# narayanan2004/GraphMat

Measured on AMD Instinct MI355X. Metric: GTEPS (edges/s) per iter + achieved HBM GB/s, PageRank RMAT-26, higher is better.
Workload: dtype f32

## Files before the change

graphmat_amd/csrc/gm_graph.hip:

```cpp
#include <string.h>
#include <cstring>

#include <hip/hip_runtime.h>
#include <rocprim/rocprim.hpp>

#include <algorithm>
#include <cmath>
#include <vector>

#include "gm_internal.hpp"

namespace gm {

int g_short_row = GM_SHORT_ROW;
int g_giant_row = 0;
int g_rank_cap = 0;
int g_rank_by = 0;
int g_tile_min_row = GM_TILE_MIN_ROW;
int g_tile_balance = 1;
int g_long_mid = 0;
int g_sweep_slices = 1;
int g_sort_tile_lists = 1;
int g_sweep_border_factor = 4;
int g_sweep_stream_weight = 300;
int g_sweep_stream = 1;
int g_sweep_waves = 16;
int g_sweep_fold_share = 50;
int g_sweep_long_row = 0;
int g_sweep_acc_limit = GM_SWEEP_ACC_ROWS, g_sweep_long_limit = GM_SWEEP_LONG_SLOTS;
int g_own_wave_row = 4096;
int g_col_tiles = 0;

constexpr int kT = 256;
inline int grid_for(int64_t n) { return (int)((n + kT - 1) / kT); }

__global__ void __launch_bounds__(kT)
k_validate_ids(const int32_t* __restrict__ src, const int32_t* __restrict__ dst, int64_t nnz, int lo, int hi,
               unsigned long long* __restrict__ bad ) {
  const int64_t e = (int64_t)blockIdx.x * kT + threadIdx.x;
  bool b = false;
  if (e < nnz) {
    const int s = src[e], d = dst[e];
    b = s < lo || s > hi || d < lo || d > hi;
  }
  const unsigned long long m = __ballot(b);
  if (m && (threadIdx.x & 63) == __ffsll((long long)m) - 1) {
    atomicAdd(&bad[0], (unsigned long long)__popcll(m));
    atomicMin(&bad[1], (unsigned long long)e + 1ull);
  }
}
// ... 1073 lines not shown
  const int W = nwaves;
  const int FW = fold_waves;
  const uint32_t g0 = grp_first[b], g1 = grp_first[b + 1] - ((skip_groups != nullptr && b < nskip_blk) ? skip_groups[b] : 0u);
  auto cost = [&](uint32_t g_) -> unsigned long long {
    const unsigned long long rows = (gbase[g_ + 1] - gbase[g_]) / 64u + 1u;
    return (gblk != nullptr && (gblk[g_] & 0x80000000u)) ? (rows * (unsigned)stream_weight + 99ull) / 100ull : rows;
  };
  unsigned long long total = 0;
  for (uint32_t g = g0; g < g1; g++) total += cost(g);
  const unsigned long long units = (unsigned long long)(W - FW) * 100ull + (unsigned long long)FW * (unsigned)fold_share;
  uint32_t g = g0;
  unsigned long long acc = 0, share = 0;
  for (int w = 0; w < W; w++) {
    wfirst[(size_t)b * (WS + 1) + w] = g;
    wrow[(size_t)b * (WS + 1) + w] = gbase[g] >> 6;
    share += w >= W - FW ? (unsigned)fold_share : 100u;
    const unsigned long long want = total * share / units;
    while (g < g1 && acc + (cost(g) + 1u) / 2u <= want) { acc += cost(g); g++; }
  }
  for (int w = W; w <= WS; w++) {
    wfirst[(size_t)b * (WS + 1) + w] = g1;
    wrow[(size_t)b * (WS + 1) + w] = gbase[g1] >> 6;
  }
}
__global__ void __launch_bounds__(kT)
k_sweep_long_starts(const unsigned long long* __restrict__ key, int64_t n, int nslices, size_t nent, uint32_t* __restrict__ lps) {
  const size_t e = (size_t)blockIdx.x * kT + threadIdx.x;
  if (e > nent) return;
  if (e == nent) { lps[e] = (uint32_t)n; return; }
  const size_t b = e / GM_SWEEP_LONG_SLOTS;
  const unsigned long long vw = b / (size_t)nslices, slice = b % (size_t)nslices, j = e % GM_SWEEP_LONG_SLOTS;
  const unsigned long long want = (vw << 23) | (slice << 16) | j;
  int64_t lo = 0, hi = n;
  while (lo < hi) { const int64_t mid = (lo + hi) >> 1; if (key[mid] >= want) hi = mid; else lo = mid + 1; }
  lps[e] = (uint32_t)lo;
}
__global__ void __launch_bounds__(kT)
k_sweep_long_fill(const unsigned long long* __restrict__ key_sorted, const uint32_t* __restrict__ pos_sorted, int64_t n, const int32_t* __restrict__ colidx,
                  const uint32_t* __restrict__ vals, SweepSlices sl, uint32_t* __restrict__ lcol, uint32_t* __restrict__ lval) {
  const int64_t i = (int64_t)blockIdx.x * kT + threadIdx.x;
  if (i >= n) return;
  const uint32_t p = pos_sorted[i];
  lcol[i] = sweep_entry_of(sl, (int)((key_sorted[i] >> 16) & 127ull), colidx[p]);
  if (lval) lval[i] = vals[p];
}
__global__ void __launch_bounds__(kT)
// ... 249 lines not shown
    GM_TRY_HIP(hipMemcpyAsync(pstart.as<uint32_t>() + npieces, &ne32, 4, hipMemcpyHostToDevice, s));
    {
      std::vector<int32_t> h(nblk + 1);
      GM_TRY_HIP(hipMemcpyAsync(h.data(), bfirst.p, (nblk + 1) * 4, hipMemcpyDeviceToHost, s));
      GM_TRY_HIP(hipStreamSynchronize(s));
      h[nblk] = (int32_t)npieces;
      for (int64_t b = (int64_t)nblk - 1; b >= 0; b--) if (h[b] < 0) h[b] = h[b + 1];
      GM_TRY_HIP(hipMemcpyAsync(bfirst.p, h.data(), (nblk + 1) * 4, hipMemcpyHostToDevice, s));
      GM_TRY_HIP(hipStreamSynchronize(s));
    }
    head.free(); pidx.free();
    DevBuf pk_in, pk_out, pid_in, sp;
    if ((rc = pk_in.alloc((size_t)npieces * 8)) || (rc = pk_out.alloc((size_t)npieces * 8)) || (rc = pid_in.alloc((size_t)npieces * 4)) || (rc = sp.alloc((size_t)npieces * 4))) return rc;
    hipLaunchKernelGGL(k_sweep_piece_keys, dim3(grid_for((int64_t)npieces)), dim3(kT), 0, s, (const uint32_t*)pstart.as<uint32_t>(), (const uint32_t*)pblk.as<uint32_t>(), npieces,
                       pk_in.as<unsigned long long>(), pid_in.as<uint32_t>());
    if ((rc = sweep_sort_pairs(pk_in.as<unsigned long long>(), pk_out.as<unsigned long long>(), pid_in.as<uint32_t>(), sp.as<uint32_t>(), (size_t)npieces,
                               16 + bits_for((uint32_t)nblk), s)))
      return rc;
    pk_in.free(); pk_out.free(); pid_in.free(); pblk.free();
    DevBuf ng, grp_first;
    if ((rc = ng.alloc((nblk + 1) * 4)) || (rc = grp_first.alloc((nblk + 1) * 4))) return rc;
    GM_TRY_HIP(hipMemsetAsync(ng.p, 0, (nblk + 1) * 4, s));
    hipLaunchKernelGGL(k_sweep_block_groups, dim3(grid_for((int64_t)nblk)), dim3(kT), 0, s, (const int32_t*)bfirst.as<int32_t>(), (int)nblk, ng.as<uint32_t>());
    if (g_sweep_stream != 0) {
      const int nsblk = 256 * TS;
      DevBuf sflag, siota, scnt, slen, kin, vin, srows_;
      DevBuf& sgroups = st_sgroups;
      if ((rc = sflag.alloc((size_t)nrows)) || (rc = siota.alloc((size_t)nrows * 4)) || (rc = st_srow.alloc((size_t)nrows * 4 + 4)) || (rc = scnt.alloc(16))) return rc;
      hipLaunchKernelGGL(k_stream_flag, dim3(grid_for(nrows)), dim3(kT), 0, s, rowptr, nrows, whole->view.short_row, sflag.as<unsigned char>());
      hipLaunchKernelGGL(k_sweep_iota, dim3(grid_for(nrows)), dim3(kT), 0, s, siota.as<int32_t>(), nrows);
      tb = 0;
      GM_TRY_HIP(rocprim::select(nullptr, tb, siota.as<int32_t>(), sflag.as<unsigned char>(), st_srow.as<int32_t>(), scnt.as<unsigned int>(), (size_t)nrows, s));
      if ((rc = tmp.alloc(tb + 256))) return rc;
      GM_TRY_HIP(rocprim::select(tmp.p, tb, siota.as<int32_t>(), sflag.as<unsigned char>(), st_srow.as<int32_t>(), scnt.as<unsigned int>(), (size_t)nrows, s));
      GM_TRY_HIP(hipMemcpyAsync(&st_nshort, scnt.p, 4, hipMemcpyDeviceToHost, s));
      GM_TRY_HIP(hipStreamSynchronize(s));
      sflag.free(); siota.free();
      if (st_nshort > 0) {
        if ((rc = slen.alloc(((size_t)st_nshort + 1) * 4)) || (rc = st_soff.alloc(((size_t)st_nshort + 1) * 4))) return rc;
        GM_TRY_HIP(hipMemsetAsync(slen.p, 0, ((size_t)st_nshort + 1) * 4, s));
        hipLaunchKernelGGL(k_sweep_lens, dim3(grid_for((int)st_nshort)), dim3(kT), 0, s, (const int32_t*)st_srow.as<int32_t>(), (int)st_nshort, rowptr, slen.as<uint32_t>());
        if ((rc = sweep_excl_scan(slen.as<uint32_t>(), st_soff.as<uint32_t>(), (size_t)st_nshort + 1, s))) return rc;
        GM_TRY_HIP(hipMemcpyAsync(&st_edges, st_soff.as<uint32_t>() + st_nshort, 4, hipMemcpyDeviceToHost, s));
        GM_TRY_HIP(hipStreamSynchronize(s));
        slen.free();
      }
      st_nbins = (int)(((unsigned long long)st_edges + GM_STREAM_BIN - 1) / GM_STREAM_BIN);
// ... 16 lines not shown
        GM_TRY_HIP(hipMemcpyAsync(&st_rows_total, st_rowbase.as<uint32_t>() + nsblk, 4, hipMemcpyDeviceToHost, s));
        hipLaunchKernelGGL(k_stream_add_groups, dim3(grid_for(nsblk)), dim3(kT), 0, s, (const uint32_t*)sgroups.as<uint32_t>(), nsblk, ng.as<uint32_t>());
        hipLaunchKernelGGL(k_stream_bin_rows, dim3(grid_for(st_nbins + 1)), dim3(kT), 0, s, (const uint32_t*)st_soff.as<uint32_t>(), (int)st_nshort, st_nbins, st_binrow.as<uint32_t>());
        hipLaunchKernelGGL(k_stream_chunks, dim3(grid_for((int64_t)st_nbins * TS)), dim3(kT), 0, s, (const unsigned long long*)st_keys.as<unsigned long long>(), st_edges, TS, st_nbins,
                           (const uint32_t*)st_first.as<uint32_t>(), (const uint32_t*)st_rowbase.as<uint32_t>(), st_chunk.as<uint32_t>());
        GM_TRY_HIP(hipGetLastError());
        GM_TRY_HIP(hipStreamSynchronize(s));
        if ((rc = st_inv.alloc((size_t)st_rows_total * 64 * 2 + 64))) return rc;
        GM_TRY_HIP(hipMemsetAsync(st_inv.p, 0xff, (size_t)st_rows_total * 64 * 2 + 64, s));
        st_built = true;
      }
    }
    if ((rc = sweep_excl_scan(ng.as<uint32_t>(), grp_first.as<uint32_t>(), nblk + 1, s))) return rc;
    GM_TRY_HIP(hipMemcpyAsync(&ngroups, grp_first.as<uint32_t>() + nblk, 4, hipMemcpyDeviceToHost, s));
    GM_TRY_HIP(hipStreamSynchronize(s));
    DevBuf gsize, gb64, gq0, gblk;
    if ((rc = gsize.alloc(((size_t)ngroups + 1) * 8)) || (rc = gb64.alloc(((size_t)ngroups + 1) * 8)) || (rc = gq0.alloc(((size_t)ngroups + 1) * 4)) ||
        (rc = gblk.alloc(((size_t)ngroups + 1) * 4)) || (rc = gbase.alloc(((size_t)ngroups + 1) * 4)))
      return rc;
    GM_TRY_HIP(hipMemsetAsync(gsize.p, 0, ((size_t)ngroups + 1) * 8, s));
    hipLaunchKernelGGL(k_sweep_group_sizes, dim3((unsigned)nblk), dim3(64), 0, s, (const int32_t*)bfirst.as<int32_t>(), (const uint32_t*)grp_first.as<uint32_t>(),
                       (const uint32_t*)sp.as<uint32_t>(), (const uint32_t*)pstart.as<uint32_t>(), gsize.as<unsigned long long>(), gq0.as<uint32_t>(), gblk.as<uint32_t>(),
                       st_built ? (const uint32_t*)st_first.as<uint32_t>() : (const uint32_t*)nullptr, 256 * TS);
    if ((rc = sweep_excl_scan(gsize.as<unsigned long long>(), gb64.as<unsigned long long>(), (size_t)ngroups + 1, s))) return rc;
    GM_TRY_HIP(hipMemcpyAsync(&nentries, gb64.as<unsigned long long>() + ngroups, 8, hipMemcpyDeviceToHost, s));
    GM_TRY_HIP(hipStreamSynchronize(s));
    if (nentries >= (1ull << 32)) return GM_OK;
    hipLaunchKernelGGL(k_sweep_narrow, dim3(grid_for((int64_t)ngroups + 1)), dim3(kT), 0, s, (const unsigned long long*)gb64.as<unsigned long long>(), (size_t)ngroups + 1,
                       gbase.as<uint32_t>());
    gsize.free(); gb64.free();
    if ((rc = scol.alloc(((size_t)nentries + 64 * 64) * 4)) || (rc = wrow.alloc(nblk * 17 * 4)) || (rc = wfirst.alloc(nblk * 17 * 4))) return rc;
    if (vals && ((rc = sval.alloc(((size_t)nentries + 64 * 64) * 4)) || (rc = spos.alloc(((size_t)nentries + 64) * 4)))) return rc;
    hipLaunchKernelGGL(k_sweep_fill, dim3(65536), dim3(kT), 0, s, ngroups, (const uint32_t*)gbase.as<uint32_t>(), (const uint32_t*)gq0.as<uint32_t>(),
                       (const uint32_t*)gblk.as<uint32_t>(), (const int32_t*)bfirst.as<int32_t>(), (const uint32_t*)sp.as<uint32_t>(), (const uint32_t*)pstart.as<uint32_t>(),
                       (const uint16_t*)pslot16.as<uint16_t>(), mpos, colidx, vals, sl, TS, (const int*)rowmin.as<int>(), scol.as<uint32_t>(),
                       vals ? sval.as<uint32_t>() : (uint32_t*)nullptr, vals ? spos.as<uint32_t>() : (uint32_t*)nullptr);
    if (st_built)
      hipLaunchKernelGGL(k_stream_fill, dim3(65536), dim3(kT), 0, s, ngroups, (const uint32_t*)gbase.as<uint32_t>(), (const uint32_t*)gq0.as<uint32_t>(),
                         (const uint32_t*)gblk.as<uint32_t>(), (const uint32_t*)st_first.as<uint32_t>(), (const uint32_t*)st_rowbase.as<uint32_t>(),
                         (const unsigned long long*)st_keys.as<unsigned long long>(), (const uint32_t*)st_idx.as<uint32_t>(), (const uint32_t*)st_spos.as<uint32_t>(), colidx, vals, sl, TS,
                         scol.as<uint32_t>(), vals ? sval.as<uint32_t>() : (uint32_t*)nullptr, vals ? spos.as<uint32_t>() : (uint32_t*)nullptr, st_inv.as<uint16_t>());
    hipLaunchKernelGGL(k_sweep_wave_ranges, dim3((unsigned)((nblk + 63) / 64)), dim3(64), 0, s, (const uint32_t*)grp_first.as<uint32_t>(), (int)nblk,
                       (const uint32_t*)gbase.as<uint32_t>(), wfirst.as<uint32_t>(), wrow.as<uint32_t>(), nlong > 0 ? g_sweep_fold_share : 100,
                       (int)std::min(8, (((per_wg_long + nsets - 1) / nsets) + 63) / 64), (g_sweep_waves == 12 || g_sweep_waves == 8) ? g_sweep_waves : 16,
                       st_built ? (const uint32_t*)st_sgroups.as<uint32_t>() : (const uint32_t*)nullptr, 256 * TS);
    if (st_built) {
      if ((rc = st_wrow.alloc(nblk * 17 * 4)) || (rc = st_wfirst.alloc(nblk * 17 * 4))) return rc;
      hipLaunchKernelGGL(k_sweep_wave_ranges, dim3((unsigned)((nblk + 63) / 64)), dim3(64), 0, s, (const uint32_t*)grp_first.as<uint32_t>(), (int)nblk,
                         (const uint32_t*)gbase.as<uint32_t>(), st_wfirst.as<uint32_t>(), st_wrow.as<uint32_t>(), nlong > 0 ? g_sweep_fold_share : 100,
                         (int)std::min(8, (((per_wg_long + nsets - 1) / nsets) + 63) / 64), 16, (const uint32_t*)nullptr, 0, (const uint32_t*)gblk.as<uint32_t>(), g_sweep_stream_weight);
    }
    GM_TRY_HIP(hipGetLastError());
    GM_TRY_HIP(hipStreamSynchronize(s));
  } else {
    if ((rc = gbase.alloc(64)) || (rc = wrow.alloc(nblk * 17 * 4)) || (rc = wfirst.alloc(nblk * 17 * 4)) || (rc = scol.alloc(64 * 64 * 4))) return rc;
    GM_TRY_HIP(hipMemsetAsync(scol.p, 0xff, 64 * 64 * 4, s));
    if (vals) {
      if ((rc = sval.alloc(64 * 64 * 4))) return rc;
      GM_TRY_HIP(hipMemsetAsync(sval.p, 0, 64 * 64 * 4, s));
    }
    GM_TRY_HIP(hipMemsetAsync(gbase.p, 0, 64, s));
    GM_TRY_HIP(hipMemsetAsync(wfirst.p, 0, nblk * 17 * 4, s));
    GM_TRY_HIP(hipMemsetAsync(wrow.p, 0, nblk * 17 * 4, s));
    GM_TRY_HIP(hipStreamSynchronize(s));
  }
  DevBuf gcol, gval, gdst, gslice, gpos;
  int64_t ngiant_edges = 0;
  if (whole->view.ngiant > 0 && whole->view.giant_edges > 0 && whole->view.giant_edges < ((int64_t)1 << 32)) {
    const int64_t ge = whole->view.giant_edges;
    DevBuf gk_in, gk_out, gp_in, gp_out, gd_in, gd_out;
    if ((rc = gk_in.alloc((size_t)ge)) || (rc = gk_out.alloc((size_t)ge)) || (rc = gp_in.alloc((size_t)ge * 4)) || (rc = gp_out.alloc((size_t)ge * 4)) ||
        (rc = gd_in.alloc((size_t)ge * 4)) || (rc = gd_out.alloc((size_t)ge * 4)) || (rc = gslice.alloc((GM_MAX_SLICES + 2) * 4)))
      return rc;
// ... 1042 lines not shown
```

graphmat_amd/csrc/gm_programs.hip:

```cpp
#include <limits.h>
#include <math.h>

#include <string>

#include "GraphMatRuntime.h"
#include "gm_internal.hpp"

#define HD __host__ __device__

namespace gm {

extern int g_short_row, g_giant_row, g_rank_by, g_rank_cap, g_col_tiles, g_tile_min_row, g_long_mid, g_tile_balance, g_own_wave_row, g_sort_tile_lists, g_sweep_slices, g_sweep_acc_limit, g_sweep_long_limit, g_sweep_long_row, g_sweep_fold_share, g_sweep_border_factor, g_blocked_rows, g_sweep_waves, g_sweep_stream, g_sweep_stream_weight;
static int g_force_ordered = 0;

struct PRv : gm_pr_t {
  HD PRv() { pagerank = 0.3; degree = 0; }
  HD int operator!=(const PRv& p) { return ((double)fabsf(p.pagerank - pagerank) > 1e-5); }
};

struct DegreeP : GraphMat::GraphProgram<int, int, PRv, int> {
  DegreeP() {
    this->order = GraphMat::IN_EDGES;
    this->process_message_requires_vertexprop = false;
  }
  HD bool send_message(const PRv&, int& message) const { message = 1; return true; }
  HD void process_message(const int& message, const int, const PRv&, int& result) const { result = message; }
  HD void reduce_function(int& a, const int& b) const { a += b; }
  HD void apply(const int& message_out, PRv& vertexprop) { vertexprop.degree = message_out; }
};

template <int ORDERED>
struct PageRankP : GraphMat::GraphProgram<float, float, PRv, int> {
  float alpha;
  explicit PageRankP(float a) : alpha(a) {
    this->activity = GraphMat::ALL_VERTICES;
// ... 687 lines not shown
  if (!g || !k || !gm::engine_value_ok(*k, value)) { gm::set_error("gm_graph_set_option: unknown engine option or value out of range"); return GM_ERR_INVALID; }
  ((int32_t*)&g->opt)[k->index] = value;
  g->opt_set |= 1u << k->index;
  return GM_OK;
}
int gm_reset_options(void) {
  gm::engine_defaults() = gm::engine_documented_defaults();
  gm::g_force_ordered = 0;
  gm::g_sgd_mfma = 0;
  gm::g_short_row = GM_SHORT_ROW;
  gm::g_giant_row = 0;
  gm::g_rank_cap = 0;
  gm::g_rank_by = 0;
  gm::g_tile_min_row = GM_TILE_MIN_ROW;
  gm::g_tile_balance = 1;
  gm::g_long_mid = 0;
  gm::g_own_wave_row = 4096;
  gm::g_sort_tile_lists = 1;
  gm::g_sweep_slices = 1;
  gm::g_blocked_rows = 0;
  gm::g_sweep_acc_limit = GM_SWEEP_ACC_ROWS;
  gm::g_sweep_long_limit = GM_SWEEP_LONG_SLOTS;
  gm::g_sweep_long_row = 0;
  gm::g_sweep_fold_share = 50;
  gm::g_sweep_waves = 16;
  gm::g_sweep_stream = 1;
  gm::g_sweep_stream_weight = 300;
  gm::g_sweep_border_factor = 4;
  gm::g_col_tiles = 0;
  return GM_OK;
}
int gm_set_option(const char* key, int value) {
  if (const gm::EngineKey* k = gm::engine_key(key)) {
    if (!gm::engine_value_ok(*k, value)) { gm::set_error("gm_set_option: value out of range"); return GM_ERR_INVALID; }
    ((int32_t*)&gm::engine_defaults())[k->index] = value;
    return GM_OK;
  }
  if (key && !strcmp(key, "force_ordered")) { gm::g_force_ordered = value; return GM_OK; }
  if (key && !strcmp(key, "sgd_mfma") && (value == 0 || value == 1)) { gm::g_sgd_mfma = value; return GM_OK; }
  if (key && !strcmp(key, "short_row") && value >= 1 && value <= GM_BLOCK_NNZ) { gm::g_short_row = value; return GM_OK; }
  if (key && !strcmp(key, "giant_row") && value >= 64) { gm::g_giant_row = value; return GM_OK; }
  if (key && !strcmp(key, "rank_cap") && value >= 0) { gm::g_rank_cap = value; return GM_OK; }
  if (key && !strcmp(key, "rank_by") && value >= 0 && value <= 2) { gm::g_rank_by = value; return GM_OK; }
  if (key && !strcmp(key, "long_mid") && value >= 0) { gm::g_long_mid = value; return GM_OK; }
  if (key && !strcmp(key, "tile_balance") && value >= 0 && value <= 100400) { gm::g_tile_balance = value; return GM_OK; }
  if (key && !strcmp(key, "tile_min_row") && (value == 0 || value >= gm::g_short_row)) { gm::g_tile_min_row = value; return GM_OK; }
  if (key && !strcmp(key, "col_tiles") && value >= 0 && value <= GM_MAX_TILES) { gm::g_col_tiles = value; return GM_OK; }
  if (key && !strcmp(key, "own_wave_row") && value >= 0) { gm::g_own_wave_row = value; return GM_OK; }
  if (key && !strcmp(key, "sort_tile_lists") && (value == 0 || value == 1)) { gm::g_sort_tile_lists = value; return GM_OK; }
  if (key && !strcmp(key, "sweep_slices") && (value == 0 || value == 1 || (value >= 8 && value <= GM_MAX_SLICES))) { gm::g_sweep_slices = value; return GM_OK; }
  if (key && !strcmp(key, "sweep_acc_rows") && value >= 1 && value <= GM_SWEEP_ACC_ROWS) { gm::g_sweep_acc_limit = value; return GM_OK; }
  if (key && !strcmp(key, "blocked_rows") && value >= -1 && value <= 1) { gm::g_blocked_rows = value; return GM_OK; }
  if (key && !strcmp(key, "sweep_long_row") && value >= 0 && value <= 8191) { gm::g_sweep_long_row = value; return GM_OK; }
  if (key && !strcmp(key, "sweep_border_factor") && value >= 1 && value <= 64) { gm::g_sweep_border_factor = value; return GM_OK; }
  if (key && !strcmp(key, "sweep_fold_share") && value >= 0 && value <= 100) { gm::g_sweep_fold_share = value; return GM_OK; }
  if (key && !strcmp(key, "sweep_stream") && (value == 0 || value == 1)) { gm::g_sweep_stream = value; return GM_OK; }
  if (key && !strcmp(key, "sweep_stream_weight") && value >= 50 && value <= 2000) { gm::g_sweep_stream_weight = value; return GM_OK; }
  if (key && !strcmp(key, "sweep_waves") && (value == 16 || value == 12 || value == 8)) { gm::g_sweep_waves = value; return GM_OK; }
  if (key && !strcmp(key, "sweep_long_slots") && value >= 1 && value <= GM_SWEEP_LONG_SLOTS) { gm::g_sweep_long_limit = value; return GM_OK; }
  gm::set_error("gm_set_option: unknown option");
  return GM_ERR_INVALID;
}

#ifdef GRAPHMAT_ABLATION
extern "C" int gm_abl_wave_times(unsigned long long* out, size_t bytes) {
  const size_t n = sizeof(GraphMat::dev::g_abl_wave_times);
  GM_TRY_HIP(hipDeviceSynchronize());
  GM_TRY_HIP(hipMemcpyFromSymbol(out, HIP_SYMBOL(GraphMat::dev::g_abl_wave_times), bytes < n ? bytes : n));
  return GM_OK;
}
#endif

int gm_debug_counters(int64_t out[4]) {
  unsigned long long h[4] = {0, 0, 0, 0};
  GM_TRY_HIP(hipMemcpyFromSymbol(h, HIP_SYMBOL(GraphMat::dev::g_longrow_counters), sizeof(h)));
  for (int i = 0; i < 4; i++) out[i] = (int64_t)h[i];
  unsigned long long z[4] = {0, 0, 0, 0};
  GM_TRY_HIP(hipMemcpyToSymbol(HIP_SYMBOL(GraphMat::dev::g_longrow_counters), z, sizeof(z)));
// ... 84 lines not shown
```

include/graphmat/engine.hpp:

```cpp
#pragma once
#include <stdio.h>
#include <stdlib.h>
#include <sys/time.h>

#include <limits>
#include <type_traits>
#include <vector>

#include "kernels.hpp"

namespace GraphMat {

enum edge_direction { OUT_EDGES, IN_EDGES, ALL_EDGES };
enum activity_type { ACTIVE_ONLY, ALL_VERTICES };

template <class T, class U, class V, class E>
class GraphProgram;

namespace detail {

template <class F>
struct member_class_of;
template <class C, class R, class... A>
struct member_class_of<R (C::*)(A...)> { typedef C type; };
// ... 1115 lines not shown
      const bool gather_apart = gterms != nullptr && sw.nsub <= 1 && ((opt.sweep_form & 16) != 0 || w12);
      auto giant_gather = [&]() {
        bool done = false;
        if constexpr (sizeof(E) == 4 && std::is_trivially_copyable<E>::value) {
          if (Aout.vals != nullptr && sw.gval != nullptr) {
            hipLaunchKernelGGL((dev::k_giant_gather_sliced<P, T, U, V, E, true>), dim3(2048), dim3(dev::kBlock), 0, aux.s, pa, sw.gcol, sw.gval, sw.gdst, (int64_t)sw.ngiant_edges, xq, gterms);
            done = true;
          }
        }
        if (!done)
          hipLaunchKernelGGL((dev::k_giant_gather_sliced<P, T, U, V, E, false>), dim3(2048), dim3(dev::kBlock), 0, aux.s, pa, sw.gcol, (const uint32_t*)nullptr, sw.gdst, (int64_t)sw.ngiant_edges, xq, gterms);
        st.spmv_launches++;
      };
      bool chain_done = false;
      if (w12 && gterms != nullptr) {
        giant_gather();
        Launch Lg = L;
        Lg.terms_ready = true;
        launch_spmv_vp<P, T, U, V, E>(use_vp, Lg, pa, Ag, xq, xb, (const V*)d_vp, y, ybits, acc, rk);
        chain_done = true;
      }
      U* sterms = nullptr;
      if (sw.nstream > 0 && sw.sinv != nullptr && sw.wrow_stream != nullptr && xb == nullptr && !w12 && !shorts_blocked && !(opt.sweep_form & 128) &&
          sw.bin_cap == GM_STREAM_BIN && (sw.nstream >= (1ll << 25) || (opt.sweep_form & 256))) {
        void* p16 = nullptr;
        if (gm_graph_workspace(g, 16, (size_t)sw.nstream_slots * sizeof(U) + 256, &p16) == GM_OK) sterms = (U*)p16;
      }
      const int where = sterms != nullptr ? 4 : shorts_blocked ? 3 : (w12 ? 1 : (gterms != nullptr ? 2 : (opt.sweep_form & 3)));
      if (where == 1) { La.s = aux.s; La.timer = nullptr; }
      auto short_rows = [&]() {
        if (As.nblk <= 0) return;
        launch_spmv_vp<P, T, U, V, E>(use_vp, La, pa, As, xq, xb, (const V*)d_vp, y, ybits, acc, rk);
        if (where == 1) { GM_HIP_OK(hipEventRecord(aux.join, aux.s)); aux.pending = true; }
      };
      if (where < 2) short_rows();
      int stage = 64;
      if (sw.nrows_long > 0) {
        stage = (sw.max_long_block + 63) / 64 * 64;
        if (stage > GM_SWEEP_MAX_STAGE) stage = GM_SWEEP_MAX_STAGE;
        if (stage < 1024) stage = 1024;
        if (opt.sweep_form & 4) stage = 1024;
      }
      if (w12 && stage > GM_SWEEP_MAX_STAGE_W12) stage = GM_SWEEP_MAX_STAGE_W12;
      for (int set = 0; set < sw.nsets; set++) {
        U* gt = (set == 0 && !gather_apart) ? gterms : (U*)nullptr;
        bool with_vals = false;
        const uint32_t* st_rows = (sterms != nullptr && set == 0) ? sw.wrow_stream : sw.wrow;
// ... 516 lines not shown
```

include/graphmat/kernels.hpp:

```cpp
#pragma once
#include <hip/hip_runtime.h>
#include <stdint.h>
#include <string.h>

#include <type_traits>

#include "../graphmat_hip.h"

namespace GraphMat {

enum reduce_kind {
  REDUCE_AUTO = -1,
  REDUCE_ORDERED = 0,
  REDUCE_COMMUTATIVE = 1,
  REDUCE_LAST = 2,
  REDUCE_F32_ADD = 3
};

template <class P>
struct program_traits {
  static constexpr reduce_kind reduce = REDUCE_AUTO;
};

template <class P>
// ... 1604 lines not shown
            const uint32_t* __restrict__ lval, const uint32_t* __restrict__ lps, const int32_t* __restrict__ lrow_of_slot,
            const uint32_t* __restrict__ gcol, const uint32_t* __restrict__ gval, const uint32_t* __restrict__ gdst, const uint32_t* __restrict__ gslice,
            U* __restrict__ gterms, const T* __restrict__ x, U* __restrict__ y) {
  sell_body<P, T, U, V, E, HAS_VALS, ABL, UBATCH, PIPE, POOLW, false>(pa, set, stage_words, nslices, nrows_long, slice_base, scol, sval, wrow, row_of_slot, lcol, lval, lps,
                                                                       lrow_of_slot, gcol, gval, gdst, gslice, gterms, x, y, 1, 0, 0);
}
template <class P, class T, class U, class V, class E, bool HAS_VALS>
__global__ void __launch_bounds__(1024)
k_spmv_sell_stream(ProgArg<P> pa, int set, int stage_words, int nslices, int nrows_long, const int32_t* __restrict__ slice_base, const uint32_t* __restrict__ scol,
                   const uint32_t* __restrict__ sval, const uint32_t* __restrict__ wrow, const int32_t* __restrict__ row_of_slot, const uint32_t* __restrict__ lcol,
                   const uint32_t* __restrict__ lval, const uint32_t* __restrict__ lps, const int32_t* __restrict__ lrow_of_slot,
                   const uint32_t* __restrict__ gcol, const uint32_t* __restrict__ gval, const uint32_t* __restrict__ gdst, const uint32_t* __restrict__ gslice,
                   U* __restrict__ gterms, const T* __restrict__ x, U* __restrict__ y, U* __restrict__ sterms) {
  sell_body<P, T, U, V, E, HAS_VALS, 0, 7, 2, GM_SWEEP_POOL, false>(pa, set, stage_words, nslices, nrows_long, slice_base, scol, sval, wrow, row_of_slot, lcol, lval, lps,
                                                                     lrow_of_slot, gcol, gval, gdst, gslice, gterms, x, y, 1, 0, 0, nullptr, nullptr, sterms);
}
template <class P, class U>
__global__ void __launch_bounds__(512, 6)
k_short_fold(ProgArg<P> pa, const U* __restrict__ sterms, const uint16_t* __restrict__ sinv, const uint32_t* __restrict__ schunk, int nslices, int cap,
             const uint32_t* __restrict__ sbin_row, const uint32_t* __restrict__ soff, const int32_t* __restrict__ srow_id, U* __restrict__ y,
             uint32_t* __restrict__ ybits) {
  static_assert(sizeof(U) == 4, "4-byte reductions");
  __shared__ uint32_t s_prod[(GM_STREAM_BIN + 64) + (GM_STREAM_BIN + 64) / 32 + 1];
  auto at = [](uint32_t q) { return q + (q >> 5); };
  __shared__ uint32_t s_cpos[GM_MAX_SLICES], s_cpre[GM_MAX_SLICES + 1];
  const P& p = *reinterpret_cast<const P*>(pa.b);
  const int b = blockIdx.x, wv = threadIdx.x >> 6, lane = threadIdx.x & 63;
  const uint32_t* __restrict__ raw = reinterpret_cast<const uint32_t*>(sterms);
  const uint32_t i0 = sbin_row[b], i1 = sbin_row[b + 1], base = (uint32_t)b * (uint32_t)cap;
  constexpr int RK = 4;
  uint32_t ro0[RK], ro1[RK];
  int rid[RK];
#pragma unroll
  for (int j = 0; j < RK; j++) {
    const uint32_t i = i0 + (uint32_t)(j * 512) + threadIdx.x;
    if (i < i1) { ro0[j] = soff[i]; ro1[j] = soff[i + 1]; rid[j] = srow_id[i]; }
  }
  if ((int)threadIdx.x < nslices) {
    const uint2 pn = *reinterpret_cast<const uint2*>(&schunk[((size_t)b * nslices + threadIdx.x) * 2]);
    s_cpos[threadIdx.x] = pn.x;
    s_cpre[threadIdx.x] = pn.y;
  }
  __syncthreads();
  constexpr int CB = 4, CK = 4;
  for (int c0 = wv; c0 < nslices; c0 += 8 * CB) {
    uint32_t vv[CB][CK];
    uint16_t qq[CB][CK];
// ... 1640 lines not shown
```

include/graphmat_hip.h:

```cpp
#ifndef GRAPHMAT_HIP_H_
#define GRAPHMAT_HIP_H_

#include <stddef.h>
#include <stdint.h>

#ifdef __cplusplus
extern "C" {
#endif

#define GM_OK 0
#define GM_ERR_INVALID 1
#define GM_ERR_HIP 2
#define GM_ERR_NOMEM 3
#define GM_ERR_UNSUPPORTED 4
#define GM_ERR_IO 5

typedef void* gm_stream_t;
typedef struct gm_graph gm_graph_t;

const char* gm_last_error(void);
int gm_version(void);
int gm_device_count(int* count);
int gm_set_device(int device);

// ... 127 lines not shown
  const uint32_t* gval;
  const uint32_t* gdst;
  const uint32_t* gslice;
  const uint32_t* gsrc_pos;
  int32_t nsub;
  int32_t stride;
  int32_t hot_words;
  int32_t waves;
  int64_t nstream;
  int64_t nstream_slots;
  int32_t nshort_rows;
  int32_t nbins;
  int32_t bin_cap;
  int32_t stream_width;
  const int32_t* srow;
  const uint32_t* soff;
  const uint32_t* sbin_row;
  const uint32_t* schunk;
  const uint16_t* sinv;
  const uint32_t* wrow_stream;
} gm_sweep_t;
#define GM_STREAM_BIN 12288
#define GM_STREAM_WIDTH 8
#define GM_SWEEP_HOT 0x40000000u
#define GM_MAX_SLICES 128
#define GM_SWEEP_ACC_ROWS 10048
#define GM_SWEEP_LONG_SLOTS 512
#define GM_SWEEP_PAD 0x80000000u
#define GM_SWEEP_POOL 30848
#define GM_SWEEP_MAX_STAGE 14336
#define GM_SWEEP_POOL_SPARSE (GM_SWEEP_POOL - 768)
#define GM_SWEEP_POOL_W12 21504
#define GM_SWEEP_MAX_STAGE_W12 9216
int gm_graph_sweep(const gm_graph_t* g, gm_sweep_t* out);
int gm_graph_tile(const gm_graph_t* g, int direction, int tile, gm_csr_t* out, const uint32_t** d_prev_bits);
typedef struct gm_blocked {
  int32_t nrows;
  int32_t nblocks;
  int32_t nslices;
  int32_t short_row;
  int32_t nsteps;
  int32_t val_bytes;
  int64_t nentries;
  const uint32_t* ecol;
  const uint16_t* erow;
  const uint32_t* woff;
// ... 129 lines not shown
```

Baseline: 330.4.

## Pack sweep groups into waves with cost-model bin packing and fold-aware caps

New measurement: 330.3 (median of 3 runs). No clear change (-0.0%).

```diff
diff --git a/graphmat_amd/csrc/gm_graph.hip b/graphmat_amd/csrc/gm_graph.hip
--- a/graphmat_amd/csrc/gm_graph.hip
+++ b/graphmat_amd/csrc/gm_graph.hip
@@ -25,7 +25,10 @@
 int g_sweep_stream_weight = 300;
 int g_sweep_stream = 1;
 int g_sweep_waves = 16;
-int g_sweep_fold_share = 50;
+int g_sweep_pack = 1;
+int g_sweep_meta_weight = 200, g_sweep_row_weight = 100, g_sweep_live_weight = 0;
+int g_sweep_fold_weight = 32;
+int g_sweep_fold_share = -1;
 int g_sweep_long_row = 0;
 int g_sweep_acc_limit = GM_SWEEP_ACC_ROWS, g_sweep_long_limit = GM_SWEEP_LONG_SLOTS;
 int g_own_wave_row = 4096;
@@ -1145,6 +1148,169 @@
     wfirst[(size_t)b * (WS + 1) + w] = g1;
     wrow[(size_t)b * (WS + 1) + w] = gbase[g1] >> 6;
   }
+}
+struct SweepCost { int meta, row, live, stream, fold; };
+__device__ __forceinline__ unsigned long long sweep_medium_cost(const SweepCost& c, uint32_t width, uint32_t live) {
+  return (unsigned long long)(unsigned)c.meta + (unsigned long long)(unsigned)c.row * width + ((unsigned long long)(unsigned)c.live * live + 63ull) / 64ull;
+}
+__device__ __forceinline__ unsigned long long sweep_stream_cost(const SweepCost& c, uint32_t width) {
+  return (((unsigned long long)(unsigned)c.meta + (unsigned long long)(unsigned)c.row * width) * (unsigned)c.stream + 99ull) / 100ull;
+}
+__global__ void __launch_bounds__(64)
+k_sweep_group_live(const int32_t* __restrict__ blk_first, const uint32_t* __restrict__ grp_first, const uint32_t* __restrict__ sp, const uint32_t* __restrict__ piece_start,
+                   uint32_t* __restrict__ live) {
+  const int b = blockIdx.x;
+  const uint32_t g0 = grp_first[b], q0 = (uint32_t)blk_first[b], qe = (uint32_t)blk_first[b + 1];
+  const uint32_t nm = (qe - q0 + 63u) / 64u;
+  for (uint32_t i = 0; i < nm; i++) {
+    const uint32_t q = q0 + i * 64u + threadIdx.x;
+    uint32_t n = 0;
+    if (q < qe) { const uint32_t p = sp[q]; n = piece_start[p + 1] - piece_start[p]; }
+    for (int o = 32; o > 0; o >>= 1) n += __shfl_down(n, o);
+    if (threadIdx.x == 0) live[g0 + i] = n;
+  }
+}
+__device__ __forceinline__ void sweep_wave_caps(unsigned long long total, int W, int FW, int fold_share, const unsigned long long* fcost, unsigned long long* cap) {
+  if (fold_share >= 0) {
+    const unsigned long long units = (unsigned long long)(W - FW) * 100ull + (unsigned long long)FW * (unsigned)fold_share;
+    for (int w = 0; w < W; w++) cap[w] = units ? (total * (w >= W - FW ? (unsigned)fold_share : 100u) + units - 1) / units : 0ull;
+    return;
+  }
+  bool off[16];
+  for (int f = 0; f < 16; f++) off[f] = false;
+  unsigned long long level = 0;
+  for (;;) {
+    unsigned long long sum = total;
+    int n = W - FW;
+    for (int f = 0; f < FW; f++) if (!off[f]) { sum += fcost[f]; n++; }
+    level = (sum + (unsigned)n - 1) / (unsigned)n;
+    bool again = false;
+    for (int f = 0; f < FW; f++) if (!off[f] && fcost[f] >= level) { off[f] = true; again = true; }
+    if (!again) break;
+  }
+  for (int w = 0; w < W; w++) {
+    const int f = W - 1 - w;
+    cap[w] = f < FW ? (off[f] ? 0ull : level - fcost[f]) : level;
+  }
+}
+__device__ __forceinline__ void sweep_cut(uint32_t g, uint32_t gend, const uint32_t* cst, int w0, int w1, const unsigned long long* avail, uint32_t* first) {
+  unsigned long long left = 0, units = 0;
+  int wl = w1 - 1;
+  for (uint32_t i = g; i < gend; i++) left += cst[i];
+  for (int w = w0; w < w1; w++) units += avail[w];
+  while (wl > w0 && avail[wl] == 0) wl--;
+  for (int w = w0; w < w1; w++) {
+    first[w] = g;
+    if (w >= wl) { g = gend; continue; }
+    const unsigned long long want = left * avail[w] / units;
+    unsigned long long acc = 0;
+    while (g < gend && acc + ((unsigned long long)cst[g] + 1ull) / 2ull <= want) { acc += cst[g]; g++; }
+    left -= acc;
+    units -= avail[w];
+  }
+}
+__global__ void __launch_bounds__(64)
+k_sweep_pack(const uint32_t* __restrict__ grp_first, const uint32_t* __restrict__ nstream_groups , int nstream_blk, int nblk,
+             const unsigned long long* __restrict__ gsize_in, const uint32_t* __restrict__ gq0_in, const uint32_t* __restrict__ live, const uint32_t* __restrict__ lps, int long_slots,
+             SweepCost c, int W, int FW, int fold_share, unsigned long long* __restrict__ gsize_out, uint32_t* __restrict__ gq0_out, uint32_t* cost,
+             uint32_t* cost_laid, uint32_t* order, unsigned char* __restrict__ wave_of, uint32_t* __restrict__ wfirst_m, uint32_t* __restrict__ wfirst_s) {
+  const int b = blockIdx.x * 64 + threadIdx.x;
+  if (b >= nblk) return;
+  constexpr int WS = 16;
+  const uint32_t g0 = grp_first[b], g1 = grp_first[b + 1];
+  const uint32_t ns = (nstream_groups != nullptr && b < nstream_blk) ? nstream_groups[b] : 0u;
+  const uint32_t nm = g1 - g0 - ns, gm = g0 + nm;
+  unsigned long long fcost[WS];
+  for (int f = 0; f < WS; f++) fcost[f] = 0ull;
+  if (FW > 0 && fold_share < 0) {
+    const uint32_t* __restrict__ lp = lps + (size_t)b * (size_t)long_slots;
+    for (int f = 0; f < FW && f * 64 < long_slots; f++) {
+      uint32_t longest = 0;
+      for (int j = f * 64; j < f * 64 + 64 && j < long_slots; j++) { const uint32_t n = lp[j + 1] - lp[j]; longest = n > longest ? n : longest; }
+      fcost[f] = ((unsigned long long)(unsigned)c.fold * longest + 63ull) / 64ull;
+    }
+  }
+  unsigned long long tm = 0, ts = 0;
+  for (uint32_t i = 0; i < nm; i++) {
+    const unsigned long long x = sweep_medium_cost(c, (uint32_t)(gsize_in[g0 + i] >> 6) - 1u, live[g0 + i]);
+    cost[g0 + i] = (uint32_t)x;
+    tm += x;
+  }
+  for (uint32_t i = gm; i < g1; i++) {
+    const unsigned long long x = sweep_stream_cost(c, (uint32_t)(gsize_in[i] >> 6) - 1u);
+    cost[i] = cost_laid[i] = (uint32_t)x;
+    ts += x;
+    gsize_out[i] = gsize_in[i];
+    gq0_out[i] = gq0_in[i];
+  }
+  for (uint32_t i = 0; i < nm; i++) {
+    const uint32_t x = cost[g0 + i];
+    uint32_t k = i;
+    while (k > 0 && cost[g0 + order[g0 + k - 1]] < x) { order[g0 + k] = order[g0 + k - 1]; k--; }
+    order[g0 + k] = i;
+  }
+  const int WP = ns > 0 ? WS : W;
+  unsigned long long cap[WS], bin[WS], load[WS];
+  uint32_t cnt[WS], fill[WS];
+  sweep_wave_caps(tm + ts, WP, FW < WP ? FW : WP - 1, fold_share, fcost, cap);
+  for (int w = 0; w < WS; w++) { bin[w] = 0; load[w] = 0; cnt[w] = 0; fill[w] = 0; }
+  int wlast = 0;
+  {
+    unsigned long long left = ts;
+    for (int w = WP - 1; w >= 0; w--) {
+      const unsigned long long take = left < cap[w] ? left : cap[w];
+      left -= take;
+      bin[w] = cap[w] - take;
+      if (bin[w] > 0 && w > wlast) wlast = w;
+    }
+  }
+  for (uint32_t k = 0; k < nm; k++) {
+    const uint32_t i = order[g0 + k];
+    int best = wlast;
+    long long room = (long long)bin[wlast] - (long long)load[wlast];
+    for (int w = wlast - 1; w >= 0; w--) {
+      const long long r = (long long)bin[w] - (long long)load[w];
+      if (bin[w] > 0 && r >= room) { room = r; best = w; }
+    }
+    wave_of[g0 + i] = (unsigned char)best;
+    load[best] += cost[g0 + i];
+    cnt[best]++;
+  }
+  uint32_t start[WS + 1];
+  start[0] = g0;
+  for (int w = 0; w < WS; w++) start[w + 1] = start[w] + cnt[w];
+  for (uint32_t k = 0; k < nm; k++) {
+    const uint32_t i = order[g0 + k];
+    const int w = wave_of[g0 + i];
+    const uint32_t at = start[w] + fill[w]++;
+    gsize_out[at] = gsize_in[g0 + i];
+    gq0_out[at] = gq0_in[g0 + i];
+    cost_laid[at] = cost[g0 + i];
+  }
+  uint32_t fs[WS + 1], fm[WS + 1];
+  for (int w = 0; w <= wlast; w++) fs[w] = start[w];
+  if (ns > 0) {
+    unsigned long long avail[WS];
+    for (int w = 0; w < WS; w++) avail[w] = cap[w];
+    avail[wlast] = cap[wlast] > load[wlast] ? cap[wlast] - load[wlast] : 0ull;
+    sweep_cut(gm, g1, cost_laid, wlast, WS, avail, fs);
+    fs[wlast] = start[wlast];
+    fs[WS] = g1;
+    sweep_wave_caps(tm, W, FW < W ? FW : W - 1, fold_share, fcost, cap);
+    sweep_cut(g0, gm, cost_laid, 0, W, cap, fm);
+    for (int w = W; w <= WS; w++) fm[w] = gm;
+  } else {
+    for (int w = wlast + 1; w <= WS; w++) fs[w] = g1;
+    for (int w = 0; w <= WS; w++) fm[w] = fs[w];
+  }
+  for (int w = 0; w <= WS; w++) {
+    wfirst_m[(size_t)b * (WS + 1) + w] = fm[w];
+    if (wfirst_s != nullptr) wfirst_s[(size_t)b * (WS + 1) + w] = fs[w];
+  }
+}
+__global__ void __launch_bounds__(kT) k_sweep_rows_of(const uint32_t* __restrict__ wfirst, size_t n, const uint32_t* __restrict__ gbase, uint32_t* __restrict__ wrow) {
+  const size_t i = (size_t)blockIdx.x * kT + threadIdx.x;
+  if (i < n) wrow[i] = gbase[wfirst[i]] >> 6;
 }
 __global__ void __launch_bounds__(kT)
 k_sweep_long_starts(const unsigned long long* __restrict__ key, int64_t n, int nslices, size_t nent, uint32_t* __restrict__ lps) {
@@ -1440,7 +1606,7 @@
     if ((rc = ng.alloc((nblk + 1) * 4)) || (rc = grp_first.alloc((nblk + 1) * 4))) return rc;
     GM_TRY_HIP(hipMemsetAsync(ng.p, 0, (nblk + 1) * 4, s));
     hipLaunchKernelGGL(k_sweep_block_groups, dim3(grid_for((int64_t)nblk)), dim3(kT), 0, s, (const int32_t*)bfirst.as<int32_t>(), (int)nblk, ng.as<uint32_t>());
-    if (g_sweep_stream != 0) {
+    if (g_sweep_stream != 0 && whole->view.short_row <= GM_STREAM_MAX_SHORT_ROW) {
       const int nsblk = 256 * TS;
       DevBuf sflag, siota, scnt, slen, kin, vin, srows_;
       DevBuf& sgroups = st_sgroups;
@@ -1503,6 +1669,32 @@
     hipLaunchKernelGGL(k_sweep_group_sizes, dim3((unsigned)nblk), dim3(64), 0, s, (const int32_t*)bfirst.as<int32_t>(), (const uint32_t*)grp_first.as<uint32_t>(),
                        (const uint32_t*)sp.as<uint32_t>(), (const uint32_t*)pstart.as<uint32_t>(), gsize.as<unsigned long long>(), gq0.as<uint32_t>(), gblk.as<uint32_t>(),
                        st_built ? (const uint32_t*)st_first.as<uint32_t>() : (const uint32_t*)nullptr, 256 * TS);
+    const int sweep_w = (g_sweep_waves == 12 || g_sweep_waves == 8) ? g_sweep_waves : 16;
+    const int fold_waves = (int)std::min(8, (((per_wg_long + nsets - 1) / nsets) + 63) / 64);
+    const bool packed = g_sweep_pack != 0;
+    if ((rc = wrow.alloc(nblk * 17 * 4)) || (rc = wfirst.alloc(nblk * 17 * 4))) return rc;
+    if (st_built && ((rc = st_wrow.alloc(nblk * 17 * 4)) || (rc = st_wfirst.alloc(nblk * 17 * 4)))) return rc;
+    if (packed) {
+      DevBuf glive, gsize2, gq02, gcost, gcost_laid, gorder, gwave;
+      const size_t n1 = (size_t)ngroups + 1;
+      if ((rc = glive.alloc(n1 * 4)) || (rc = gsize2.alloc(n1 * 8)) || (rc = gq02.alloc(n1 * 4)) || (rc = gcost.alloc(n1 * 4)) || (rc = gcost_laid.alloc(n1 * 4)) ||
+          (rc = gorder.alloc(n1 * 4)) || (rc = gwave.alloc(n1)))
+        return rc;
+      GM_TRY_HIP(hipMemsetAsync(gsize2.p, 0, n1 * 8, s));
+      GM_TRY_HIP(hipMemsetAsync(glive.p, 0, n1 * 4, s));
+      hipLaunchKernelGGL(k_sweep_group_live, dim3((unsigned)nblk), dim3(64), 0, s, (const int32_t*)bfirst.as<int32_t>(), (const uint32_t*)grp_first.as<uint32_t>(),
+                         (const uint32_t*)sp.as<uint32_t>(), (const uint32_t*)pstart.as<uint32_t>(), glive.as<uint32_t>());
+      const SweepCost sc = {g_sweep_meta_weight, g_sweep_row_weight, g_sweep_live_weight, g_sweep_stream_weight, g_sweep_fold_weight};
+      hipLaunchKernelGGL(k_sweep_pack, dim3((unsigned)((nblk + 63) / 64)), dim3(64), 0, s, (const uint32_t*)grp_first.as<uint32_t>(),
+                         st_built ? (const uint32_t*)st_sgroups.as<uint32_t>() : (const uint32_t*)nullptr, 256 * TS, (int)nblk, (const unsigned long long*)gsize.as<unsigned long long>(),
+                         (const uint32_t*)gq0.as<uint32_t>(), (const uint32_t*)glive.as<uint32_t>(), (const uint32_t*)lps.as<uint32_t>(), (int)GM_SWEEP_LONG_SLOTS, sc, sweep_w,
+                         nlong > 0 ? fold_waves : 0, g_sweep_fold_share, gsize2.as<unsigned long long>(), gq02.as<uint32_t>(), gcost.as<uint32_t>(), gcost_laid.as<uint32_t>(),
+                         gorder.as<uint32_t>(), gwave.as<unsigned char>(), wfirst.as<uint32_t>(), st_built ? st_wfirst.as<uint32_t>() : (uint32_t*)nullptr);
+      GM_TRY_HIP(hipGetLastError());
+      GM_TRY_HIP(hipStreamSynchronize(s));
+      std::swap(gsize.p, gsize2.p);
+      std::swap(gq0.p, gq02.p);
+    }
     if ((rc = sweep_excl_scan(gsize.as<unsigned long long>(), gb64.as<unsigned long long>(), (size_t)ngroups + 1, s))) return rc;
     GM_TRY_HIP(hipMemcpyAsync(&nentries, gb64.as<unsigned long long>() + ngroups, 8, hipMemcpyDeviceToHost, s));
     GM_TRY_HIP(hipStreamSynchronize(s));
@@ -1510,7 +1702,7 @@
     hipLaunchKernelGGL(k_sweep_narrow, dim3(grid_for((int64_t)ngroups + 1)), dim3(kT), 0, s, (const unsigned long long*)gb64.as<unsigned long long>(), (size_t)ngroups + 1,
                        gbase.as<uint32_t>());
     gsize.free(); gb64.free();
-    if ((rc = scol.alloc(((size_t)nentries + 64 * 64) * 4)) || (rc = wrow.alloc(nblk * 17 * 4)) || (rc = wfirst.alloc(nblk * 17 * 4))) return rc;
+    if ((rc = scol.alloc(((size_t)nentries + 64 * 64) * 4))) return rc;
     if (vals && ((rc = sval.alloc(((size_t)nentries + 64 * 64) * 4)) || (rc = spos.alloc(((size_t)nentries + 64) * 4)))) return rc;
     hipLaunchKernelGGL(k_sweep_fill, dim3(65536), dim3(kT), 0, s, ngroups, (const uint32_t*)gbase.as<uint32_t>(), (const uint32_t*)gq0.as<uint32_t>(),
                        (const uint32_t*)gblk.as<uint32_t>(), (const int32_t*)bfirst.as<int32_t>(), (const uint32_t*)sp.as<uint32_t>(), (const uint32_t*)pstart.as<uint32_t>(),
@@ -1521,15 +1713,21 @@
                          (const uint32_t*)gblk.as<uint32_t>(), (const uint32_t*)st_first.as<uint32_t>(), (const uint32_t*)st_rowbase.as<uint32_t>(),
                          (const unsigned long long*)st_keys.as<unsigned long long>(), (const uint32_t*)st_idx.as<uint32_t>(), (const uint32_t*)st_spos.as<uint32_t>(), colidx, vals, sl, TS,
                          scol.as<uint32_t>(), vals ? sval.as<uint32_t>() : (uint32_t*)nullptr, vals ? spos.as<uint32_t>() : (uint32_t*)nullptr, st_inv.as<uint16_t>());
-    hipLaunchKernelGGL(k_sweep_wave_ranges, dim3((unsigned)((nblk + 63) / 64)), dim3(64), 0, s, (const uint32_t*)grp_first.as<uint32_t>(), (int)nblk,
-                       (const uint32_t*)gbase.as<uint32_t>(), wfirst.as<uint32_t>(), wrow.as<uint32_t>(), nlong > 0 ? g_sweep_fold_share : 100,
-                       (int)std::min(8, (((per_wg_long + nsets - 1) / nsets) + 63) / 64), (g_sweep_waves == 12 || g_sweep_waves == 8) ? g_sweep_waves : 16,
-                       st_built ? (const uint32_t*)st_sgroups.as<uint32_t>() : (const uint32_t*)nullptr, 256 * TS);
-    if (st_built) {
-      if ((rc = st_wrow.alloc(nblk * 17 * 4)) || (rc = st_wfirst.alloc(nblk * 17 * 4))) return rc;
+    if (packed) {
+      hipLaunchKernelGGL(k_sweep_rows_of, dim3(grid_for((int64_t)nblk * 17)), dim3(kT), 0, s, (const uint32_t*)wfirst.as<uint32_t>(), nblk * 17, (const uint32_t*)gbase.as<uint32_t>(),
+                         wrow.as<uint32_t>());
+      if (st_built)
+        hipLaunchKernelGGL(k_sweep_rows_of, dim3(grid_for((int64_t)nblk * 17)), dim3(kT), 0, s, (const uint32_t*)st_wfirst.as<uint32_t>(), nblk * 17,
+                           (const uint32_t*)gbase.as<uint32_t>(), st_wrow.as<uint32_t>());
+    } else {
+      const int former_share = nlong > 0 ? (g_sweep_fold_share >= 0 ? g_sweep_fold_share : 50) : 100;
       hipLaunchKernelGGL(k_sweep_wave_ranges, dim3((unsigned)((nblk + 63) / 64)), dim3(64), 0, s, (const uint32_t*)grp_first.as<uint32_t>(), (int)nblk,
-                         (const uint32_t*)gbase.as<uint32_t>(), st_wfirst.as<uint32_t>(), st_wrow.as<uint32_t>(), nlong > 0 ? g_sweep_fold_share : 100,
-                         (int)std::min(8, (((per_wg_long + nsets - 1) / nsets) + 63) / 64), 16, (const uint32_t*)nullptr, 0, (const uint32_t*)gblk.as<uint32_t>(), g_sweep_stream_weight);
+                         (const uint32_t*)gbase.as<uint32_t>(), wfirst.as<uint32_t>(), wrow.as<uint32_t>(), former_share, fold_waves, sweep_w,
+                         st_built ? (const uint32_t*)st_sgroups.as<uint32_t>() : (const uint32_t*)nullptr, 256 * TS);
+      if (st_built)
+        hipLaunchKernelGGL(k_sweep_wave_ranges, dim3((unsigned)((nblk + 63) / 64)), dim3(64), 0, s, (const uint32_t*)grp_first.as<uint32_t>(), (int)nblk,
+                           (const uint32_t*)gbase.as<uint32_t>(), st_wfirst.as<uint32_t>(), st_wrow.as<uint32_t>(), former_share, fold_waves, 16, (const uint32_t*)nullptr, 0,
+                           (const uint32_t*)gblk.as<uint32_t>(), g_sweep_stream_weight);
     }
     GM_TRY_HIP(hipGetLastError());
     GM_TRY_HIP(hipStreamSynchronize(s));
diff --git a/graphmat_amd/csrc/gm_programs.hip b/graphmat_amd/csrc/gm_programs.hip
--- a/graphmat_amd/csrc/gm_programs.hip
+++ b/graphmat_amd/csrc/gm_programs.hip
@@ -10,7 +10,7 @@
 
 namespace gm {
 
-extern int g_short_row, g_giant_row, g_rank_by, g_rank_cap, g_col_tiles, g_tile_min_row, g_long_mid, g_tile_balance, g_own_wave_row, g_sort_tile_lists, g_sweep_slices, g_sweep_acc_limit, g_sweep_long_limit, g_sweep_long_row, g_sweep_fold_share, g_sweep_border_factor, g_blocked_rows, g_sweep_waves, g_sweep_stream, g_sweep_stream_weight;
+extern int g_short_row, g_giant_row, g_rank_by, g_rank_cap, g_col_tiles, g_tile_min_row, g_long_mid, g_tile_balance, g_own_wave_row, g_sort_tile_lists, g_sweep_slices, g_sweep_acc_limit, g_sweep_long_limit, g_sweep_long_row, g_sweep_fold_share, g_sweep_border_factor, g_blocked_rows, g_sweep_waves, g_sweep_stream, g_sweep_stream_weight, g_sweep_pack, g_sweep_meta_weight, g_sweep_row_weight, g_sweep_live_weight, g_sweep_fold_weight;
 static int g_force_ordered = 0;
 
 struct PRv : gm_pr_t {
@@ -744,7 +744,12 @@
   gm::g_sweep_acc_limit = GM_SWEEP_ACC_ROWS;
   gm::g_sweep_long_limit = GM_SWEEP_LONG_SLOTS;
   gm::g_sweep_long_row = 0;
-  gm::g_sweep_fold_share = 50;
+  gm::g_sweep_fold_share = -1;
+  gm::g_sweep_pack = 1;
+  gm::g_sweep_meta_weight = 200;
+  gm::g_sweep_row_weight = 100;
+  gm::g_sweep_live_weight = 0;
+  gm::g_sweep_fold_weight = 32;
   gm::g_sweep_waves = 16;
   gm::g_sweep_stream = 1;
   gm::g_sweep_stream_weight = 300;
@@ -775,7 +780,12 @@
   if (key && !strcmp(key, "blocked_rows") && value >= -1 && value <= 1) { gm::g_blocked_rows = value; return GM_OK; }
   if (key && !strcmp(key, "sweep_long_row") && value >= 0 && value <= 8191) { gm::g_sweep_long_row = value; return GM_OK; }
   if (key && !strcmp(key, "sweep_border_factor") && value >= 1 && value <= 64) { gm::g_sweep_border_factor = value; return GM_OK; }
-  if (key && !strcmp(key, "sweep_fold_share") && value >= 0 && value <= 100) { gm::g_sweep_fold_share = value; return GM_OK; }
+  if (key && !strcmp(key, "sweep_fold_share") && value >= -1 && value <= 100) { gm::g_sweep_fold_share = value; return GM_OK; }
+  if (key && !strcmp(key, "sweep_pack") && (value == 0 || value == 1)) { gm::g_sweep_pack = value; return GM_OK; }
+  if (key && !strcmp(key, "sweep_meta_weight") && value >= 0 && value <= 2000) { gm::g_sweep_meta_weight = value; return GM_OK; }
+  if (key && !strcmp(key, "sweep_row_weight") && value >= 1 && value <= 2000) { gm::g_sweep_row_weight = value; return GM_OK; }
+  if (key && !strcmp(key, "sweep_live_weight") && value >= 0 && value <= 2000) { gm::g_sweep_live_weight = value; return GM_OK; }
+  if (key && !strcmp(key, "sweep_fold_weight") && value >= 0 && value <= 2000) { gm::g_sweep_fold_weight = value; return GM_OK; }
   if (key && !strcmp(key, "sweep_stream") && (value == 0 || value == 1)) { gm::g_sweep_stream = value; return GM_OK; }
   if (key && !strcmp(key, "sweep_stream_weight") && value >= 50 && value <= 2000) { gm::g_sweep_stream_weight = value; return GM_OK; }
   if (key && !strcmp(key, "sweep_waves") && (value == 16 || value == 12 || value == 8)) { gm::g_sweep_waves = value; return GM_OK; }
diff --git a/include/graphmat/engine.hpp b/include/graphmat/engine.hpp
--- a/include/graphmat/engine.hpp
+++ b/include/graphmat/engine.hpp
@@ -1161,7 +1161,7 @@
       }
       U* sterms = nullptr;
       if (sw.nstream > 0 && sw.sinv != nullptr && sw.wrow_stream != nullptr && xb == nullptr && !w12 && !shorts_blocked && !(opt.sweep_form & 128) &&
-          sw.bin_cap == GM_STREAM_BIN && (sw.nstream >= (1ll << 25) || (opt.sweep_form & 256))) {
+          sw.bin_cap == GM_STREAM_BIN && sw.short_row <= GM_STREAM_MAX_SHORT_ROW  && (sw.nstream >= (1ll << 25) || (opt.sweep_form & 256))) {
         void* p16 = nullptr;
         if (gm_graph_workspace(g, 16, (size_t)sw.nstream_slots * sizeof(U) + 256, &p16) == GM_OK) sterms = (U*)p16;
       }
diff --git a/include/graphmat/kernels.hpp b/include/graphmat/kernels.hpp
--- a/include/graphmat/kernels.hpp
+++ b/include/graphmat/kernels.hpp
@@ -1650,7 +1650,8 @@
              uint32_t* __restrict__ ybits) {
   static_assert(sizeof(U) == 4, "4-byte reductions");
   __shared__ uint32_t s_prod[(GM_STREAM_BIN + 64) + (GM_STREAM_BIN + 64) / 32 + 1];
-  auto at = [](uint32_t q) { return q + (q >> 5); };
+  static_assert(GM_STREAM_BIN + 64 >= GM_STREAM_BIN - 1 + GM_STREAM_MAX_SHORT_ROW, "k_short_fold: a bin's products (its rows start below GM_STREAM_BIN; the last may have GM_STREAM_MAX_SHORT_ROW) must fit s_prod");
+  auto at =[](uint32_t q) { return q + (q >> 5); };
   __shared__ uint32_t s_cpos[GM_MAX_SLICES], s_cpre[GM_MAX_SLICES + 1];
   const P& p = *reinterpret_cast<const P*>(pa.b);
   const int b = blockIdx.x, wv = threadIdx.x >> 6, lane = threadIdx.x & 63;
diff --git a/include/graphmat_hip.h b/include/graphmat_hip.h
--- a/include/graphmat_hip.h
+++ b/include/graphmat_hip.h
@@ -173,6 +173,7 @@
 } gm_sweep_t;
 #define GM_STREAM_BIN 12288
 #define GM_STREAM_WIDTH 8
+#define GM_STREAM_MAX_SHORT_ROW 64
 #define GM_SWEEP_HOT 0x40000000u
 #define GM_MAX_SLICES 128
 #define GM_SWEEP_ACC_ROWS 10048
```
